# waffcloud/sitewhere

Hardware: AMD Instinct MI355X
Metric: device_events_per_sec (higher is better)
Workload: dtype fp64/int64 (event values as in the reference; no reduced precision)

## Files before the change

### csrc/hip/swgpu.hip

```cpp
#include <hip/hip_runtime.h>
#include <hsa/hsa.h>
#include <hsa/hsa_ext_amd.h>
#include <stdint.h>
#include "swtypes.h"
#include "swdecode.h"
#include "swengine.h"
#include "swseg.h"
#include "swblock.h"

#define BLK 256
#define WAVES (BLK / 64)
#define TILE_ITEMS 4
#define TILE (BLK * TILE_ITEMS)
#define MAX_GRID 2048
#define STAGE_BYTES (32 * 1024)
#define MAX_PROBE 4096

#ifndef SW_XCD_REMAP
#define SW_XCD_REMAP 0
#endif
__device__ __forceinline__ uint32_t sw_block_id() {
#if SW_XCD_REMAP
  const uint32_t nwg = gridDim.x, orig = blockIdx.x, x = orig % 8u, q = nwg / 8u, r = nwg % 8u;
  return (x < r ? x * (q + 1u) : r * (q + 1u) + (x - r) * q) + orig / 8u;
// ... 114 lines not shown
    uint32_t tc, tv;
    const uint32_t pc = block_excl_scan(e ? 1u : 0u, &tc, lds);
    const uint32_t pv = block_excl_scan(v, &tv, lds);
    if (e && run_c + pc < n_msgs) {
      const uint32_t off = run_v + pv;
      msg_off[run_c + pc] = off < raw_bytes ? off : raw_bytes;
    }
    run_c += tc;
    run_v += tv;
  }
}

__device__ __forceinline__ bool stage_window(const uint8_t* __restrict__ raw, const uint32_t* __restrict__ off,
                                             int64_t n_msgs, uint8_t* lds, uint32_t* base_abs) {
  const int64_t m0 = (int64_t)BID * BLK;
  int64_t m1 = m0 + BLK;
  if (m1 > n_msgs) m1 = n_msgs;
  const uint32_t s = off[m0], e = off[m1];
  const uint32_t a0 = s & ~15u;
  const uint32_t span = e - a0;
  if (span > STAGE_BYTES) return false;
  const uint32_t nvec = (span + 15) >> 4;
  const uint4* src = reinterpret_cast<const uint4*>(raw + a0);
  uint4* dst = reinterpret_cast<uint4*>(lds);
  for (uint32_t v = threadIdx.x; v < nvec; v += BLK) dst[v] = src[v];
  __syncthreads();
  *base_abs = a0;
  return true;
}

#define CNT_ERR 0x80000000u
#define CNT_OVR 0x40000000u

__global__ __launch_bounds__(BLK) void k_decode_count(const uint8_t* __restrict__ raw, const uint32_t* __restrict__ off,
                                                      int64_t n_msgs, uint32_t* __restrict__ cnt,
                                                      uint32_t* __restrict__ tsum, SwEngineArgs a) {
  __shared__ __attribute__((aligned(16))) uint8_t lds[STAGE_BYTES];
  if (BID == 0 && threadIdx.x == 0) {
    *a.n_new_names = 0;
    *a.overflow = 0;
    ((ull*)a.stats)[SW_STAT_MSGS] += (ull)a.n_msgs;
  }
  uint32_t base = 0;
  const bool staged = stage_window(raw, off, n_msgs, lds, &base);
  __shared__ uint32_t red[WAVES + 1];
  const int64_t m = (int64_t)BID * BLK + threadIdx.x;
  uint32_t c = 0;
  if (m < n_msgs) {
    uint32_t verdict = SW_DEC_UNKNOWN;
    c = staged ? sw_decode_payload(lds, off[m] - base, off[m + 1] - base, base, 0, 0, nullptr, 0, &verdict)
               : sw_decode_payload(raw, off[m], off[m + 1], 0, 0, 0, nullptr, 0, &verdict);
    cnt[m] = c | (verdict == SW_DEC_ERROR ? CNT_ERR : 0u) | (verdict == SW_DEC_OVERSIZE ? CNT_OVR : 0u);
  }
  uint32_t tot;
  block_excl_scan(c, &tot, red);
  if (threadIdx.x == 0) tsum[BID] = tot;
}

__device__ __forceinline__ void note_name(const SwEventRec& r, ull* __restrict__ key, int64_t mask,
                                          SwNameRef* __restrict__ list, uint32_t* __restrict__ n_list, int64_t cap) {
  if (r.name_hash == 0 || r.etype >= 16) return;
  const ull h = r.name_hash;
  int64_t slot = (int64_t)(h & (ull)mask);
  for (int64_t p = 0; p <= mask && p < MAX_PROBE; ++p) {
    ull old = key[slot];
    if (old == h) return;
    if (old == 0) {
      old = atomicCAS(&key[slot], 0ull, h);
      if (old == 0) {
        const uint32_t k = atomicAdd(n_list, 1u);
        if (k < cap) {
          SwNameRef ref;
          ref.hash = h; ref.off = r.aux_off; ref.len = r.aux_len; ref.src_rank = r.src_rank; ref.pad = r.etype;
          list[k] = ref;
        } else {
          atomicExch(&key[slot], 0ull);
        }
        return;
      }
      if (old == h) return;
    }
    slot = (slot + 1) & mask;
  }
}

__global__ __launch_bounds__(BLK) void k_decode_emit(SwEngineArgs a) {
  __shared__ __attribute__((aligned(16))) uint8_t lds[STAGE_BYTES];
  uint32_t base = 0;
  const bool staged = stage_window(a.raw, a.msg_off, a.n_msgs, lds, &base);
  __shared__ uint32_t red[WAVES + 1];
  const int64_t m = (int64_t)BID * BLK + threadIdx.x;
  uint32_t tot;
  const uint32_t cv = m < a.n_msgs ? a.msg_cnt[m] : 0u;
  const uint32_t pre = block_excl_scan(cv & ~(CNT_ERR | CNT_OVR), &tot, red);
  const uint32_t blk_off = block_sum_prefix(a.msg_evoff, BID, red);
  if (BID == 0) {
    const uint32_t all = block_sum_prefix(a.msg_evoff, gridDim.x, red);
    if (threadIdx.x == 0) *a.n_recs = all;
  }
  if (m >= a.n_msgs) return;
  uint32_t verdict = (cv & CNT_ERR) ? SW_DEC_ERROR : (cv & CNT_OVR) ? SW_DEC_OVERSIZE : SW_DEC_VALID;
  const int64_t o = (int64_t)blk_off + pre;
  if (o >= a.rec_cap) return;
  const uint32_t room = (uint32_t)((a.rec_cap - o) < 0xffffffffll ? (a.rec_cap - o) : 0xffffffffll);
  SwEventRec* out = a.recs + o;
  uint32_t n;
  SwStrRef* sp = a.spans ? a.spans + o : nullptr;
  if (staged)
    n = sw_decode_payload(lds, a.msg_off[m] - base, a.msg_off[m + 1] - base, base, a.now_ms, (uint8_t)a.rank, out, room,
                          &verdict, sp);
  else
    n = sw_decode_payload(a.raw, a.msg_off[m], a.msg_off[m + 1], 0, a.now_ms, (uint8_t)a.rank, out, room, &verdict, sp);
  for (uint32_t k = 0; k < n && k < room; ++k)
    note_name(out[k], (ull*)a.seen_key, a.seen_mask, a.new_names, a.n_new_names, a.names_cap);
}

__global__ void k_decode_end(SwEngineArgs a) {
  if (threadIdx.x == 0 && BID == 0) {
    if (*a.n_recs > a.rec_cap) *a.n_recs = (uint32_t)a.rec_cap;
    ((ull*)a.stats)[SW_STAT_NEW_NAMES] += *a.n_new_names;
  }
}

__device__ __forceinline__ uint32_t part_dest(const SwEngineArgs& a, const SwEventRec& r, uint32_t world,
                                              uint32_t rank) {
  if (r.etype >= 16) return rank;
  int64_t slot = (int64_t)(r.fp_lo & (ull)a.reg_mask);
  for (int64_t p = 0; p <= a.reg_mask && p < MAX_PROBE; ++p) {
    const ulonglong2 k = *reinterpret_cast<const ulonglong2*>(&a.reg[slot].lo);
    if (k.x == r.fp_lo && k.y == r.fp_hi) return a.reg[slot].asg >= 0 ? sw_owner(r.fp_hi, world) : rank;
    if (k.x == 0 && k.y == 0) break;
    slot = (slot + 1) & a.reg_mask;
  }
  return rank;
}

// ... 1095 lines not shown
    run += tot;
  }
}

__global__ void k_presence(SwEngineArgs a) {
  const SwStepParams P = *a.sp;
  if (P.presence_missing_ms <= 0) return;
  const ull limit = (ull)(P.now_ms - P.presence_missing_ms);
  for (int64_t s = (int64_t)BID * BLK + threadIdx.x; s < a.n_asg; s += (int64_t)gridDim.x * BLK) {
    SwAsgState* st = &a.st[s];
    const ull last = st->last;
    const bool miss = last != 0 && last < limit && st->missing == 0 && a.asg_active[s];
    if (!miss) continue;
    st->missing = (ull)P.now_ms;
    const uint32_t g = atomicAdd(a.n_gen, 1u);
    if (g < a.gen_cap) {
      SwEventRec r;
      r.fp_lo = 0; r.fp_hi = 0; r.event_date = P.now_ms; r.name_hash = a.presence_name_hash;
      r.v0 = 0; r.v1 = 0; r.v2 = 0; r.alt_hash = 0;
      r.aux_off = 0; r.aux2_off = 0; r.aux_len = 0; r.aux2_len = 0;
      r.etype = SW_EV_STATE_CHANGE; r.flags = 0; r.src_rank = (uint8_t)a.rank; r.level = 0;
      a.gen[g] = r;
      a.gen_dev[g] = a.asg_ctx[s].device;
      a.gen_asg[g] = (int32_t)s;
    }
  }
}

__global__ void k_decode_begin(SwEngineArgs a) {
  if (threadIdx.x == 0 && BID == 0) {
    *a.n_new_names = 0;
    *a.overflow = 0;
    ((ull*)a.stats)[SW_STAT_MSGS] += (ull)a.n_msgs;
  }
}

__global__ void k_gen_clamp(SwEngineArgs a, uint32_t* gen_rules) {
  if (threadIdx.x == 0 && BID == 0) {
    if (*a.n_gen > a.gen_cap) *a.n_gen = (uint32_t)a.gen_cap;
    if (gen_rules) *gen_rules = *a.n_gen;
  }
}

__global__ void k_step_end(SwEngineArgs a, const uint32_t* n_rule_alerts) {
  if (threadIdx.x == 0 && BID == 0) {
    if (*a.n_gen > a.gen_cap) *a.n_gen = (uint32_t)a.gen_cap;
    *a.store_cursor += (int64_t)*a.n_ok + *a.n_gen;
    *a.n_out = (uint32_t)(*a.store_cursor - *a.step_cursor0);
    *a.seq_base += *a.n_work;
    ull* st = (ull*)a.stats;
    st[SW_STAT_EVENTS] += *a.n_work;
    st[SW_STAT_PERSISTED] += *a.n_out;
    st[SW_STAT_RULE_ALERTS] += *n_rule_alerts;
    st[SW_STAT_PRESENCE] += *a.n_gen - *n_rule_alerts;
    int64_t* meta = a.dd_meta;
    if (meta[2] == 1) {
      meta[0] ^= 1;
      meta[1] = 0;
      meta[2] = 2;
    }
    meta[3] = 0;
    if (a.dd_ff && a.dd_ff_meta[6] >= a.dd_ff_meta[2]) {
      int64_t* fm = a.dd_ff_meta;
      fm[0] = (fm[0] + 1) % a.dd_ff_gens;
      fm[SW_FF_META + fm[0]] = *a.store_cursor;
      fm[6] = 0;
// ... 769 lines not shown
  return n > 0 ? (int)hipMemcpyAsync(dst, src, (size_t)n, hipMemcpyHostToDevice, s) : 0;
}
int sw_memset_async(void* dst, int32_t v, int64_t n, hipStream_t s) {
  return n > 0 ? (int)hipMemsetAsync(dst, v, (size_t)n, s) : 0;
}

int sw_step_snapshot(const uint32_t* scalars, const uint32_t* seg_meta, const uint32_t* rej_cnt,
                     const uint32_t* n_carry, int32_t produced, SwStepSnapshot* host, hipStream_t s) {
  k_step_snapshot<<<1, 64, 0, s>>>(scalars, seg_meta, rej_cnt, n_carry, produced, host);
  return (int)hipGetLastError();
}

int sw_frame_varint(const uint8_t* lens, int64_t nbytes, int64_t n_msgs, uint32_t* msg_off, uint32_t raw_bytes,
                    uint32_t* tmp, int64_t tmp_len, hipStream_t s) {
  int64_t nt = (nbytes + TILE - 1) / TILE;
  if (nt < 1) nt = 1;
  if (2 * nt > tmp_len) return -2;
  if (nbytes <= 0 || n_msgs <= 0) return (int)hipMemsetAsync(msg_off, 0, sizeof(uint32_t) * (n_msgs + 1), s);
  uint32_t* tcnt = tmp;
  uint32_t* tlen = tmp + nt;
  k_vlen_tiles<<<(unsigned)nt, BLK, 0, s>>>(lens, nbytes, tcnt, tlen);
  k_vlen_apply<<<(unsigned)nt, BLK, 0, s>>>(lens, nbytes, tcnt, tlen, msg_off, n_msgs, raw_bytes);
  return (int)hipGetLastError();
}

int sw_phase_decode(const SwEngineArgs* ap, hipStream_t s) {
  const SwEngineArgs a = *ap;
  if (a.n_msgs <= 0) {
    k_decode_begin<<<1, 64, 0, s>>>(a);
    (void)hipMemsetAsync(a.n_recs, 0, sizeof(uint32_t), s);
    return (int)hipGetLastError();
  }
  const unsigned nb = (unsigned)((a.n_msgs + BLK - 1) / BLK);
  k_decode_count<<<nb, BLK, 0, s>>>(a.raw, a.msg_off, a.n_msgs, a.msg_cnt, a.msg_evoff, a);
  k_decode_emit<<<nb, BLK, 0, s>>>(a);
  if (a.world > 1) k_decode_end<<<1, 64, 0, s>>>(a);
  return (int)hipGetLastError();
}

int sw_phase_partition(const SwEngineArgs* ap, hipStream_t s) {
  const SwEngineArgs a = *ap;
  const int64_t ntiles = (a.carry_cap + a.rec_cap + TILE - 1) / TILE;
  if (a.world > 64 || ntiles * a.world > a.part_tmp_len || !a.carry || !a.n_carry || !a.spill || !a.n_spill ||
      a.carry == a.spill || !a.part_owner || !a.part_bytes || !a.part_meta || ntiles >= 0x7fffffff)
    return -3;
  if (a.send_str && (!a.part_len || !a.carry_spans || !a.carry_str || !a.spill_spans || !a.spill_str ||
                     a.carry_str == a.spill_str || a.carry_str_cap <= 0 || a.carry_str_cap > 0xffffffffll ||
                     a.str_cap > 0x7fffffffll))
    return -4;
  k_part_count<<<(unsigned)ntiles, BLK, 0, s>>>(a.carry, a.n_carry, a.recs, a.n_recs, (int)a.world, (int)a.rank,
                                                a.part_tmp, ntiles, a);
  int rc = launch_scan(a.part_tmp, ntiles * a.world, a.part_tmp + ntiles * a.world, nullptr, a.scan_tmp,
                       a.scan_tmp_len, s);
  if (rc) return rc;
  const uint32_t* toff = a.part_tmp + ntiles * a.world;
  k_part_cut<<<(unsigned)a.world, BLK, 0, s>>>(toff, a.part_tmp, ntiles, a.n_carry, a.n_recs, a);
  k_part_write<<<(unsigned)ntiles, BLK, 0, s>>>(a.carry, a.n_carry, a.recs, a.n_recs, (int)a.world, (int)a.rank, toff,
                                                a.part_tmp, ntiles, a.send, a.shuf_cap, a.spill, a.carry_cap, a);
  k_part_counts<<<1, 64, 0, s>>>(toff, a.part_tmp, ntiles, (int)a.world, a);
  return (int)hipGetLastError();
}

int sw_phase_unpack(const SwEngineArgs* ap, hipStream_t s) {
  const SwEngineArgs a = *ap;
  if (a.work_str && (a.str_cap & 15)) return -5;
  k_unpack<<<grid_for(a.rec_cap), BLK, 0, s>>>(a.recv, a.recv_cnt, (int)a.world, a.shuf_cap, a.work, a.n_work,
                                               a.rec_cap, a);
  return (int)hipGetLastError();
}

// ... 464 lines not shown
```

### csrc/include/swdecode.h

```cpp
#pragma once
#include "swtypes.h"

SW_HD void sw_fill_control(SwEventRec* r, uint8_t etype, uint32_t abs_start, uint32_t abs_end,
                           uint64_t lo, uint64_t hi, int64_t now_ms, uint8_t src_rank) {
  r->fp_lo = lo; r->fp_hi = hi; r->event_date = now_ms; r->name_hash = 0;
  r->v0 = 0; r->v1 = 0; r->v2 = 0; r->alt_hash = 0;
  r->aux_off = abs_start; r->aux2_off = abs_end; r->aux_len = 0; r->aux2_len = 0;
  r->etype = etype; r->flags = 0; r->src_rank = src_rank; r->level = 0;
}

SW_HD void sw_clear_span(SwStrRef* s) {
  s->alt_off = 0; s->meta_off = 0; s->alt_len = 0; s->meta_len = 0; s->k = 0; s->has = 0; s->pad = 0;
}

SW_HD bool sw_read_tag(const uint8_t* buf, uint32_t* pos, uint32_t end, uint32_t* f, uint32_t* wt) {
  uint64_t key;
  if (!sw_read_varint(buf, pos, end, &key) || key > 0xffffffffull || (key >> 3) == 0) return false;
  *f = (uint32_t)(key >> 3);
  *wt = (uint32_t)(key & 7);
  return true;
}

SW_HD bool sw_check_pair(const uint8_t* buf, uint32_t* pos, uint32_t end, uint32_t wt2, uint32_t* len1 = nullptr) {
  uint64_t len;
  if (!sw_read_varint(buf, pos, end, &len) || len > (uint64_t)(end - *pos)) return false;
  uint32_t p = *pos;
  const uint32_t e = p + (uint32_t)len;
  bool h1 = false, h2 = false;
  while (p < e) {
    uint32_t f, wt;
    if (!sw_read_tag(buf, &p, e, &f, &wt)) return false;
    const uint32_t vs = p;
    if (!sw_skip_field(buf, &p, e, wt)) return false;
    if (f == 1 && wt == 2) {
      h1 = true;
      if (len1) {
        uint32_t q = vs;
        uint64_t l;
        sw_read_varint(buf, &q, e, &l);
        if ((uint32_t)l > *len1) *len1 = (uint32_t)l;
      }
    }
    h2 |= f == 2 && wt == wt2;
  }
  *pos = e;
  return h1 && h2;
}

#define SW_DEC_UNKNOWN 0u
#define SW_DEC_VALID 1u
#define SW_DEC_ERROR 2u
#define SW_DEC_OVERSIZE 3u
SW_HD uint32_t sw_decode_payload(const uint8_t* buf, uint32_t start, uint32_t end, uint32_t abs_base,
                                 int64_t now_ms, uint8_t src_rank, SwEventRec* out, uint32_t max_out,
                                 uint32_t* verdict = nullptr, SwStrRef* spans = nullptr) {
  const uint32_t known = verdict ? *verdict : SW_DEC_UNKNOWN;
  if (out && known == SW_DEC_ERROR) {
    if (max_out) {
      sw_fill_control(out, SW_EV_DECODE_ERROR, abs_base + start, abs_base + end, 0, 0, now_ms, src_rank);
      if (spans) sw_clear_span(spans);
    }
    return 1;
  }
  const bool trusted = out && known == SW_DEC_VALID;
  uint32_t pos = start;
  uint64_t hlen = 0, blen = 0, v = 0;
  uint64_t cmd = 0;
  bool ok = sw_read_varint(buf, &pos, end, &hlen) && hlen <= (uint64_t)(end - pos);
  if (ok) {
    uint32_t hend = pos + (uint32_t)hlen;
    while (ok && pos < hend) {
      uint32_t f, wt;
      ok = sw_read_tag(buf, &pos, hend, &f, &wt);
      if (!ok) break;
      if (f == 1 && wt == 0) {
        ok = sw_read_varint(buf, &pos, hend, &v);
        if (v >= 1 && v <= 8) cmd = v;
      } else {
        ok = sw_skip_field(buf, &pos, hend, wt);
      }
    }
    ok = ok && sw_read_varint(buf, &pos, end, &blen) && blen <= (uint64_t)(end - pos);
  }
  if (!ok || cmd < 1 || cmd > 8) {
    if (out && max_out) {
      sw_fill_control(out, SW_EV_DECODE_ERROR, abs_base + start, abs_base + end, 0, 0, now_ms, src_rank);
      if (spans) sw_clear_span(spans);
    }
    if (!out && verdict) *verdict = SW_DEC_ERROR;
    return 1;
  }
  const uint32_t bstart = pos, bend = pos + (uint32_t)blen;
  const bool event = cmd == SW_CMD_SEND_DEVICE_MEASUREMENTS || cmd == SW_CMD_SEND_DEVICE_LOCATION ||
                     cmd == SW_CMD_SEND_DEVICE_ALERT;
  const uint32_t meta_f = cmd == SW_CMD_SEND_DEVICE_MEASUREMENTS ? 4u : cmd == SW_CMD_SEND_DEVICE_LOCATION ? 6u : 5u;

  uint64_t lo = 0, hi = 0, date = 0;
  bool has_dev = false, has_date = false, has_us = false, us = false, has_elev = false, has_alt = false;
  bool req_a = false, req_b = false;
  uint32_t n_mx = 0, name_max = 0;
  double lat = 0, lon = 0, elev = 0;
  uint32_t t_off = start, t_len = 0, m_off = start, m_len = 0;
  uint32_t a_off = start, a_len = 0;
  uint32_t md_lo = 0, md_hi = 0;
  bool has_md = false;
  pos = bstart;
  while (ok && pos < bend) {
    uint32_t f, wt;
    const uint32_t fstart = pos;
    ok = sw_read_tag(buf, &pos, bend, &f, &wt);
    if (!ok) break;
    if (f == 1 && wt == 2) {
      ok = sw_read_varint(buf, &pos, bend, &v) && v <= (uint64_t)(bend - pos);
      if (!ok) break;
      if (out) sw_fingerprint(buf + pos, (uint32_t)v, &lo, &hi);
      has_dev = true;
      pos += (uint32_t)v;
      continue;
    }
    if (f == SW_FIELD_ALTERNATE_ID && wt == 2 && event) {
      ok = sw_read_varint(buf, &pos, bend, &v) && v <= (uint64_t)(bend - pos);
      if (!ok) break;
      a_off = pos; a_len = (uint32_t)v; has_alt = true;
      pos += (uint32_t)v;
      continue;
    }
    if (event && f == meta_f && wt == 2) {
      ok = trusted ? sw_skip_field(buf, &pos, bend, wt) : sw_check_pair(buf, &pos, bend, 2);
      if (!has_md) md_lo = fstart;
      md_hi = pos;
      has_md = true;
      continue;
    }
    switch (cmd) {
      case SW_CMD_SEND_DEVICE_MEASUREMENTS:
        if (f == 2 && wt == 2) { n_mx++; ok = trusted ? sw_skip_field(buf, &pos, bend, wt) : sw_check_pair(buf, &pos, bend, 1, &name_max); }
        else if (f == 3 && wt == 1) { if (pos + 8 > bend) { ok = false; break; } date = sw_load_le64(buf + pos); pos += 8; has_date = true; }
        else if (f == 5 && wt == 0) { ok = sw_read_varint(buf, &pos, bend, &v); has_us = true; us = v != 0; }
        else ok = sw_skip_field(buf, &pos, bend, wt);
        break;
      case SW_CMD_SEND_DEVICE_LOCATION:
        if ((f == 2 || f == 3 || f == 4 || f == 5) && wt == 1) {
          if (pos + 8 > bend) { ok = false; break; }
          uint64_t bits = sw_load_le64(buf + pos); pos += 8;
          double d;
          __builtin_memcpy(&d, &bits, 8);
          if (f == 2) { lat = d; req_a = true; } else if (f == 3) { lon = d; req_b = true; }
          else if (f == 4) { elev = d; has_elev = true; }
          else { date = bits; has_date = true; }
        } else if (f == 7 && wt == 0) { ok = sw_read_varint(buf, &pos, bend, &v); has_us = true; us = v != 0; }
        else ok = sw_skip_field(buf, &pos, bend, wt);
        break;
      case SW_CMD_SEND_DEVICE_ALERT:
        if ((f == 2 || f == 3) && wt == 2) {
          ok = sw_read_varint(buf, &pos, bend, &v) && v <= (uint64_t)(bend - pos);
          if (!ok) break;
          if (f == 2) { t_off = pos; t_len = (uint32_t)v; req_a = true; } else { m_off = pos; m_len = (uint32_t)v; req_b = true; }
          pos += (uint32_t)v;
        } else if (f == 4 && wt == 1) { if (pos + 8 > bend) { ok = false; break; } date = sw_load_le64(buf + pos); pos += 8; has_date = true; }
        else if (f == 6 && wt == 0) { ok = sw_read_varint(buf, &pos, bend, &v); has_us = true; us = v != 0; }
        else ok = sw_skip_field(buf, &pos, bend, wt);
        break;
      default:
        ok = sw_skip_field(buf, &pos, bend, wt);
        break;
    }
  }
  if ((cmd == SW_CMD_SEND_DEVICE_LOCATION || cmd == SW_CMD_SEND_DEVICE_ALERT) && !(req_a && req_b)) ok = false;
  if (!ok || !has_dev) {
    if (!out && verdict) *verdict = SW_DEC_ERROR;
    if (out && max_out) {
      sw_fill_control(out, SW_EV_DECODE_ERROR, abs_base + start, abs_base + end, 0, 0, now_ms, src_rank);
      if (spans) sw_clear_span(spans);
    }
    return 1;
  }
  const bool oversize = event && (known == SW_DEC_OVERSIZE ||
                                  (!trusted && (a_len > 0xffffu || md_hi - md_lo > 0xffffu || t_len > 0xffffu ||
                                                m_len > 0xffffu || name_max > 0xffffu)));
  if (oversize) {
    if (!out && verdict) *verdict = SW_DEC_OVERSIZE;
    if (!out) return 1;
    if (!max_out) return 0;
    sw_fill_control(out, SW_EV_OVERSIZE, abs_base + start, abs_base + end, lo, hi, now_ms, src_rank);
    if (spans) sw_clear_span(spans);
    return 1;
  }
  uint8_t flags = (has_us ? SW_F_HAS_UPDATE_STATE : 0) | (us ? SW_F_UPDATE_STATE : 0) |
                  (has_date ? SW_F_HAS_DATE : 0) | (has_elev ? SW_F_HAS_ELEVATION : 0);
  int64_t edate = has_date ? (int64_t)date : now_ms;
  SwStrRef sp;
  sp.alt_off = abs_base + a_off; sp.alt_len = (uint16_t)a_len;
  sp.meta_off = has_md ? abs_base + md_lo : abs_base + start; sp.meta_len = has_md ? (uint16_t)(md_hi - md_lo) : 0;
  sp.k = 0; sp.has = (has_alt ? SW_SR_ALT : 0) | (has_md ? SW_SR_META : 0); sp.pad = 0;

  if (!out && verdict) *verdict = SW_DEC_VALID;
  if (!out) return cmd == SW_CMD_SEND_DEVICE_MEASUREMENTS ? n_mx : 1;
  const uint64_t alt = has_alt && (cmd != SW_CMD_SEND_DEVICE_MEASUREMENTS || n_mx == 1) ? sw_hash64(buf + a_off, a_len) : 0;
  if (cmd == SW_CMD_SEND_DEVICE_MEASUREMENTS) {
    if (n_mx > max_out) {
      if (max_out) {
        sw_fill_control(out, SW_EV_DECODE_ERROR, abs_base + start, abs_base + end, lo, hi, now_ms, src_rank);
        if (spans) sw_clear_span(spans);
      }
      return max_out ? 1 : 0;
    }
    const bool multi = n_mx > 1;
    uint32_t k = 0;
    pos = bstart;
    while (pos < bend && k < n_mx) {
      uint64_t key;
      if (!sw_read_varint(buf, &pos, bend, &key)) break;
      uint32_t f = (uint32_t)(key >> 3), wt = (uint32_t)(key & 7);
      if (!(f == 2 && wt == 2)) { if (!sw_skip_field(buf, &pos, bend, wt)) break; continue; }
      sw_read_varint(buf, &pos, bend, &v);
      uint32_t mend = pos + (uint32_t)v;
      uint32_t n_off = start, n_len = 0;
      double val = 0;
      while (pos < mend) {
        uint64_t k2;
        if (!sw_read_varint(buf, &pos, mend, &k2)) { pos = mend; break; }
        uint32_t f2 = (uint32_t)(k2 >> 3), w2 = (uint32_t)(k2 & 7);
        if (f2 == 1 && w2 == 2) {
          uint64_t l2;
          if (!sw_read_varint(buf, &pos, mend, &l2) || l2 > (uint64_t)(mend - pos)) { pos = mend; break; }
          n_off = pos; n_len = (uint32_t)l2; pos += (uint32_t)l2;
        } else if (f2 == 2 && w2 == 1 && pos + 8 <= mend) {
          uint64_t bits = sw_load_le64(buf + pos); pos += 8;
          __builtin_memcpy(&val, &bits, 8);
        } else if (!sw_skip_field(buf, &pos, mend, w2)) { pos = mend; break; }
      }
      pos = mend;
      SwEventRec* r = out + k;
      r->fp_lo = lo; r->fp_hi = hi; r->event_date = edate;
      r->name_hash = n_len ? sw_hash64(buf + n_off, n_len) : 0;
      r->v0 = val; r->v1 = 0; r->v2 = 0;
      r->alt_hash = !has_alt ? 0 : multi ? sw_hash64_sfx(buf + a_off, a_len, k) : alt;
      r->aux_off = abs_base + n_off; r->aux2_off = 0;
      r->aux_len = (uint16_t)n_len; r->aux2_len = 0;
      r->etype = SW_EV_MEASUREMENT; r->flags = flags; r->src_rank = src_rank; r->level = 0;
      if (spans) {
        spans[k] = sp;
        spans[k].k = (uint16_t)(k > 0xffffu ? 0xffffu : k);
        spans[k].has |= multi ? SW_SR_MULTI : 0;
      }
      ++k;
    }
    for (; k < n_mx; ++k) {
      sw_fill_control(out + k, SW_EV_DECODE_ERROR, abs_base + start, abs_base + end, lo, hi, now_ms, src_rank);
      if (spans) sw_clear_span(spans + k);
    }
    return n_mx;
  }
  if (!max_out) return 0;
  if (spans) *spans = sp;
  if (cmd == SW_CMD_SEND_DEVICE_LOCATION) {
    out->fp_lo = lo; out->fp_hi = hi; out->event_date = edate; out->name_hash = 0;
    out->v0 = lat; out->v1 = lon; out->v2 = elev; out->alt_hash = alt;
    out->aux_off = abs_base + start; out->aux2_off = 0; out->aux_len = 0; out->aux2_len = 0;
    out->etype = SW_EV_LOCATION; out->flags = flags; out->src_rank = src_rank; out->level = 0;
    return 1;
  }
  if (cmd == SW_CMD_SEND_DEVICE_ALERT) {
    out->fp_lo = lo; out->fp_hi = hi; out->event_date = edate;
    out->name_hash = t_len ? sw_hash64(buf + t_off, t_len) : 0;
    out->v0 = 0; out->v1 = 0; out->v2 = 0; out->alt_hash = alt;
    out->aux_off = abs_base + t_off; out->aux2_off = abs_base + m_off;
    out->aux_len = (uint16_t)t_len;
    out->aux2_len = (uint16_t)m_len;
    out->etype = SW_EV_ALERT; out->flags = flags; out->src_rank = src_rank; out->level = 0;
    return 1;
  }
  if (spans) sw_clear_span(spans);
  uint8_t et = cmd == SW_CMD_SEND_REGISTRATION ? SW_EV_REGISTRATION
             : cmd == SW_CMD_SEND_ACKNOWLEDGEMENT ? SW_EV_ACK
             : cmd == SW_CMD_SEND_DEVICE_STREAM ? SW_EV_STREAM_CREATE
             : cmd == SW_CMD_SEND_DEVICE_STREAM_DATA ? SW_EV_STREAM_DATA
             : SW_EV_STREAM_DATA_REQUEST;
  sw_fill_control(out, et, abs_base + start, abs_base + end, lo, hi, now_ms, src_rank);
  return 1;
}
```

### sitewhere_amd/_native.py

```python
from __future__ import annotations

import ctypes
import os
import shutil
import subprocess
import threading
from pathlib import Path

ROOT = Path(__file__).resolve().parent.parent
LIB_DIR = Path(__file__).resolve().parent / "_lib"
CSRC = ROOT / "csrc"
GPU_ARCH = os.environ.get("SW_GPU_ARCH", "gfx950")

_NATIVE_SRC = [CSRC / "native" / "swnative.cpp", CSRC / "native" / "swcpuengine.cpp", CSRC / "native" / "swseg.cpp",
               CSRC / "native" / "swindex.cpp", CSRC / "native" / "swroute.cpp", CSRC / "native" / "swsandbox.cpp", CSRC / "native" / "swjson.cpp",
               CSRC / "native" / "swrowjson.cpp"]
_GPU_SRC = [CSRC / "hip" / "swgpu.hip", CSRC / "hip" / "swseg.hip", CSRC / "hip" / "swindex.hip"]
_HEADERS = sorted((CSRC / "include").glob("*.h")) + sorted((CSRC / "hip").glob("*.h"))

_lock = threading.Lock()
_native = None
_gpu = None


# ... 222 lines not shown
            _proto(lib, "swlog_append_routed", c_int64, P, P, P, c_int64, P, P, c_int64, P)
            _proto(lib, "swlog_append", c_int64, P, c_int32, c_int32, P, c_int64, P, c_int64, c_int64)
            _proto(lib, "swlog_end_offset", c_int64, P, c_int32, c_int32)
            _proto(lib, "swlog_begin_offset", c_int64, P, c_int32, c_int32)
            _proto(lib, "swlog_read", c_int64, P, c_int32, c_int32, c_int64, c_int64, P, c_int64, P)
            _proto(lib, "swlog_commit", c_int32, P, c_char_p, c_int32, c_int32, c_int64)
            _proto(lib, "swlog_committed", c_int64, P, c_char_p, c_int32, c_int32)
            _proto(lib, "swlog_append_external", c_int64, P, c_int32, c_int32, P, c_int64, c_int64, c_int64,
                   c_int64)
            _proto(lib, "swlog_view", c_int32, P, c_int32, c_int32, c_int64, P, P, P)
            _proto(lib, "swlog_hold", c_int32, P, c_int32, c_int32, c_int64)
            _proto(lib, "swlog_take_released", c_int64, P, P, c_int64)
            _proto(lib, "sw_partition_for_key", c_int32, c_char_p, c_int32, c_int32)
            _native_gil = lib
    return _native_gil


def gpu():
    global _gpu
    if _gpu is not None:
        return _gpu
    import torch

    with _lock:
        if _gpu is not None:
            return _gpu
        override = os.environ.get("SW_GPU_LIB")
        path = Path(override) if override else LIB_DIR / "libswgpu.so"
        if not override and _stale(path, _GPU_SRC):
            build_gpu()
        lib = ctypes.CDLL(str(path))
        P = c_void_p
        _proto(lib, "sw_phase_decode", c_int32, P, P)
        _proto(lib, "sw_phase_partition", c_int32, P, P)
        _proto(lib, "sw_phase_unpack", c_int32, P, P)
        _proto(lib, "sw_phase_process", c_int32, P, P, P)
        _proto(lib, "sw_pip_batch", c_int32, P, c_int64, P, P, c_int64, P, P)
        _proto(lib, "sw_store_filter", c_int32, P, c_int32, P, c_int64, P, P)
        _proto(lib, "sw_store_series_count", c_int32, P, P, P, P)
        _proto(lib, "sw_store_series", c_int32, P, P, P, c_int64, P, P, c_int64, P, P, P, P, P)
        _proto(lib, "sw_store_near", c_int32, P, P, P, c_int64, P, P)
        _proto(lib, "sw_store_zone", c_int32, P, P, c_int64, P, P)
        _proto(lib, "sw_store_grid", c_int32, P, P, P, P)
        _proto(lib, "sw_grid_lds_cells", c_int64, c_int64)
        _proto(lib, "sw_store_rank", c_int32, P, P, P, P, P, P)
        _proto(lib, "sw_rank_lds_keys", c_int64, c_int64)
        _proto(lib, "sw_rank_combine", c_int32, c_int32)
        _proto(lib, "sw_scan_u32", c_int32, P, c_int64, P, P, P, c_int64, P)
        _proto(lib, "sw_state_lookup", c_int32, P, c_int64, c_int32, c_int32, P, P, P)
        _proto(lib, "sw_abi_sizes", c_int32, P)
        _proto(lib, "sw_host_alloc", c_int32, c_int64, P, P)
        _proto(lib, "sw_host_free", c_int32, P)
        _proto(lib, "sw_push_out", c_int32, P, P, P, c_int64, c_int32, P)
        _proto(lib, "sw_copy_d2h", c_int32, P, P, c_int64, P)
        _proto(lib, "sw_sdma_copy", c_int32, P, P, c_int64, c_int32, ctypes.POINTER(ctypes.c_uint64))
        _proto(lib, "sw_sdma_h2d", c_int32, P, P, c_int64, c_int32, ctypes.POINTER(ctypes.c_uint64))
        _proto(lib, "sw_frame_varint", c_int32, P, c_int64, c_int64, P, ctypes.c_uint32, P, c_int64, P)
        _proto(lib, "sw_set_step_params", c_int32, P, c_int64, c_int64, c_int64, P, P, c_int64, P)
        _proto(lib, "sw_graph_capture_process", c_int32, P, P, c_int32, P, ctypes.POINTER(ctypes.c_void_p))
        _proto(lib, "sw_graph_launch", c_int32, P, P)
        _proto(lib, "sw_graph_destroy", c_int32, P)
        _proto(lib, "sw_sdma_wait", c_int32, c_uint64)
        _proto(lib, "sw_seg_encode", c_int32, P, P, P, P, P, c_int64, P, c_int64, P)
        _proto(lib, "sw_seg_encode_stamped", c_int32, P, P, P, P, P, c_int64, P, c_int64, P, P)
        _proto(lib, "sw_seg_encode_snap", c_int32, P, P, P, P, P, c_int64, P, c_int64, P, P, P, P, P)
        _proto(lib, "sw_seg_aux", c_int32, P, P, P, P, P, c_int64, P, P, c_int64, P)
# ... 52 lines not shown
```

### sitewhere_amd/pipeline/gpu_engine.py

```python
from __future__ import annotations

import ctypes
import functools
import os
import time

import numpy as np
import torch

from .._native import gpu_gil as gpu_lib
from ..models.columnar import (EVENT_REC, RANK_CELL, RANK_QUERY, GRID_CELL, GRID_QUERY_F64, GRID_WORDS, N_STATS, NEAR_QUERY, NEAR_QUERY_F64,
                               OUT_REC, NAME_REF, OUT_REC_SIZE, RING_QUERY, SC_N_GEN, SC_N_NEW_NAMES, SC_N_OK, SC_N_OUT,
                               SC_N_RECS, SC_N_REJ, SC_N_RULE, SC_N_WORK, SC_NAMES, SC_OVERFLOW, SEG_ST_BYTES, SEG_ST_FIRST, SEG_ST_WORDS, SERIES_CELL, SERIES_QUERY,
                               ST_RECHECK, STEP_SNAPSHOT, STR_REF, WIRE_REC, ZONE_QUERY, ZONE_QUERY_F64)
from ..ops.engine_abi import SwEngineArgs
from .config import EngineConfig
from .bus_io import host_view
from .engine_base import EngineBase, StepResult
from .pinned_pool import PinnedPool

_ALIGN = 64
_I64 = np.iinfo(np.int64)


# ... 565 lines not shown

    def string_drops(self) -> dict:
        v = self.t["str_drops"].cpu().numpy()
        return {"oversize": int(v[0])}

    def scalars(self) -> dict:
        v = self.t["scalars"][:len(SC_NAMES)].cpu().numpy()
        return {name: int(x) for name, x in zip(SC_NAMES, v)}

    def step(self, raw: np.ndarray, offs: np.ndarray, now_ms: int, presence: bool | None = None) -> StepResult:
        n_msgs = len(offs) - 1
        with self._lock:
            self._no_framed_pending()
            raw_dev, off_dev = self._stage(raw, offs)
            do_presence = self.presence_due(now_ms) if presence is None else presence
            sel = self.step_async(raw_dev, off_dev, n_msgs, now_ms, presence=do_presence, out_to_device=True)
            self._sync_streams()
            return self._with_block(self.collect(sel, raw, from_device=True), sel, now_ms)

    def decode_only(self, raw: np.ndarray, offs: np.ndarray, now_ms: int, spans: bool = False):
        n_msgs = len(offs) - 1
        with self._lock:
            self._no_framed_pending()
            raw_dev, off_dev = self._stage(raw, offs)
            self._set_batch(raw_dev, off_dev, n_msgs, now_ms)
            _chk(self.lib.sw_phase_decode(ctypes.byref(self.args), self._stream()), "sw_phase_decode")
            self._sync_streams()
            n = min(int(self.t["scalars"][SC_N_RECS].item()), self.cfg.rec_cap)
            recs = self.t["recs"][:n * EVENT_REC.itemsize].cpu().numpy().view(EVENT_REC).copy()
            if not spans:
                return recs
            return recs, self.t["spans"][:n * STR_REF.itemsize].cpu().numpy().view(STR_REF).copy()

    def step_framed(self, batch, now_ms: int, presence: bool | None = None) -> StepResult:
        if batch.lens is None:
            return EngineBase.step_framed(self, batch, now_ms, presence)
        import warnings
        n, nb, nl = batch.n_msgs, len(batch.payload), len(batch.lens)
        if n > self.cfg.max_msgs:
            raise ValueError(f"batch of {n} payloads exceeds EngineConfig.max_msgs={self.cfg.max_msgs}")
        if nb < batch.payload_bytes + _ALIGN:
            raise ValueError("raw batch payload lacks its tail padding")
        with self._lock:
            self._no_framed_pending()
            dev_r, dev_l, dev_o = self._stg_framed.get(nb, nl)
            with warnings.catch_warnings():
                warnings.simplefilter("ignore", UserWarning)
                pt = torch.frombuffer(batch.payload, dtype=torch.uint8) if nb else None
                lt = torch.frombuffer(batch.lens, dtype=torch.uint8) if nl else None
            if pt is not None:
                dev_r[:nb].copy_(pt, non_blocking=True)
            if lt is not None:
                dev_l[:nl].copy_(lt, non_blocking=True)
            self.frame_varint(dev_l, nl, n, dev_o, batch.payload_bytes)
            do_presence = self.presence_due(now_ms) if presence is None else presence
            sel = self.step_async(dev_r[:nb], dev_o[:n + 1], n, now_ms, presence=do_presence, out_to_device=True)
            self._sync_streams()
            return self._with_block(self.collect(sel, np.asarray(batch.payload), from_device=True), sel, now_ms)

    encode_blocks = False
    block_boot = 0

    def _with_block(self, res: StepResult, sel: int, now_ms: int) -> StepResult:
        if self.encode_blocks:
            res.block = self.encode_block(now_ms, res, slot=sel, boot=self.block_boot)
        return res
# ... 1125 lines not shown
```

Before: 536.5 million.

## Speculatively emit single-event records in decode count pass to skip re-decode

Splits the payload decoder into a parse step and an emit step. When the previous batch produced one event per message (tracked through a flag word in device memory), the first pass writes each record directly at index m. The second pass then re-decodes only the messages whose final offset differs, and skips LDS staging for blocks with no remaining work. This avoids decoding every payload twice in the common case. In exchange it adds an extra begin kernel launch, flag bookkeeping across batches, and wasted speculative writes when the batch is mixed.

```diff
diff --git a/csrc/hip/swgpu.hip b/csrc/hip/swgpu.hip
--- a/csrc/hip/swgpu.hip
+++ b/csrc/hip/swgpu.hip
@@ -170,29 +170,10 @@
 #define CNT_ERR 0x80000000u
 #define CNT_OVR 0x40000000u
 
-__global__ __launch_bounds__(BLK) void k_decode_count(const uint8_t* __restrict__ raw, const uint32_t* __restrict__ off,
-                                                      int64_t n_msgs, uint32_t* __restrict__ cnt,
-                                                      uint32_t* __restrict__ tsum, SwEngineArgs a) {
-  __shared__ __attribute__((aligned(16))) uint8_t lds[STAGE_BYTES];
-  if (BID == 0 && threadIdx.x == 0) {
-    *a.n_new_names = 0;
-    *a.overflow = 0;
-    ((ull*)a.stats)[SW_STAT_MSGS] += (ull)a.n_msgs;
-  }
-  uint32_t base = 0;
-  const bool staged = stage_window(raw, off, n_msgs, lds, &base);
-  __shared__ uint32_t red[WAVES + 1];
-  const int64_t m = (int64_t)BID * BLK + threadIdx.x;
-  uint32_t c = 0;
-  if (m < n_msgs) {
-    uint32_t verdict = SW_DEC_UNKNOWN;
-    c = staged ? sw_decode_payload(lds, off[m] - base, off[m + 1] - base, base, 0, 0, nullptr, 0, &verdict)
-               : sw_decode_payload(raw, off[m], off[m + 1], 0, 0, 0, nullptr, 0, &verdict);
-    cnt[m] = c | (verdict == SW_DEC_ERROR ? CNT_ERR : 0u) | (verdict == SW_DEC_OVERSIZE ? CNT_OVR : 0u);
-  }
-  uint32_t tot;
-  block_excl_scan(c, &tot, red);
-  if (threadIdx.x == 0) tsum[BID] = tot;
+#define SPEC_CUR_OFF 1u
+#define SPEC_NEXT_OFF 2u
+__device__ __forceinline__ bool decode_speculates(const SwEngineArgs& a) {
+  return a.str_drops && !(__atomic_load_n(&a.str_drops[1], __ATOMIC_RELAXED) & SPEC_CUR_OFF);
 }
 
 __device__ __forceinline__ void note_name(const SwEventRec& r, ull* __restrict__ key, int64_t mask,
@@ -222,24 +203,69 @@
   }
 }
 
-__global__ __launch_bounds__(BLK) void k_decode_emit(SwEngineArgs a) {
+__global__ __launch_bounds__(BLK) void k_decode_first(const uint8_t* __restrict__ raw, const uint32_t* __restrict__ off,
+                                                      int64_t n_msgs, uint32_t* __restrict__ cnt,
+                                                      uint32_t* __restrict__ tsum, SwEngineArgs a) {
   __shared__ __attribute__((aligned(16))) uint8_t lds[STAGE_BYTES];
+  const bool spec = decode_speculates(a);
   uint32_t base = 0;
-  const bool staged = stage_window(a.raw, a.msg_off, a.n_msgs, lds, &base);
+  const bool staged = stage_window(raw, off, n_msgs, lds, &base);
   __shared__ uint32_t red[WAVES + 1];
   const int64_t m = (int64_t)BID * BLK + threadIdx.x;
+  uint32_t c = 0;
+  if (!spec) {
+    if (m < n_msgs) {
+      uint32_t verdict = SW_DEC_UNKNOWN;
+      c = staged ? sw_decode_payload(lds, off[m] - base, off[m + 1] - base, base, 0, 0, nullptr, 0, &verdict)
+                 : sw_decode_payload(raw, off[m], off[m + 1], 0, 0, 0, nullptr, 0, &verdict);
+      cnt[m] = c | (verdict == SW_DEC_ERROR ? CNT_ERR : 0u) | (verdict == SW_DEC_OVERSIZE ? CNT_OVR : 0u);
+    }
+  } else if (m < n_msgs) {
+    uint32_t verdict = SW_DEC_UNKNOWN;
+    SwEventRec* out = m < a.rec_cap ? a.recs + m : nullptr;
+    SwStrRef* sp = out && a.spans ? a.spans + m : nullptr;
+    c = staged ? sw_decode_once(lds, off[m] - base, off[m + 1] - base, base, a.now_ms, (uint8_t)a.rank, out, &verdict, sp)
+               : sw_decode_once(raw, off[m], off[m + 1], 0, a.now_ms, (uint8_t)a.rank, out, &verdict, sp);
+    cnt[m] = c | (verdict == SW_DEC_ERROR ? CNT_ERR : 0u) | (verdict == SW_DEC_OVERSIZE ? CNT_OVR : 0u);
+    if (out && c == 1) note_name(*out, (ull*)a.seen_key, a.seen_mask, a.new_names, a.n_new_names, a.names_cap);
+  }
+  uint32_t tot;
+  block_excl_scan(c, &tot, red);
+  if (threadIdx.x == 0) tsum[BID] = tot;
+}
+
+__global__ __launch_bounds__(BLK) void k_decode_second(SwEngineArgs a) {
+  __shared__ __attribute__((aligned(16))) uint8_t lds[STAGE_BYTES];
+  __shared__ uint32_t red[WAVES + 1];
+  const int64_t m = (int64_t)BID * BLK + threadIdx.x;
+  const bool spec = decode_speculates(a);
+  uint32_t base = 0;
+  bool staged = false;
+  if (!spec) staged = stage_window(a.raw, a.msg_off, a.n_msgs, lds, &base);
   uint32_t tot;
   const uint32_t cv = m < a.n_msgs ? a.msg_cnt[m] : 0u;
-  const uint32_t pre = block_excl_scan(cv & ~(CNT_ERR | CNT_OVR), &tot, red);
+  const uint32_t c = cv & ~(CNT_ERR | CNT_OVR);
+  const uint32_t pre = block_excl_scan(c, &tot, red);
   const uint32_t blk_off = block_sum_prefix(a.msg_evoff, BID, red);
   if (BID == 0) {
     const uint32_t all = block_sum_prefix(a.msg_evoff, gridDim.x, red);
-    if (threadIdx.x == 0) *a.n_recs = all;
-  }
-  if (m >= a.n_msgs) return;
+    if (threadIdx.x == 0) {
+      *a.n_recs = all;
+      if (a.str_drops) {
+        const uint32_t w = __atomic_load_n(&a.str_drops[1], __ATOMIC_RELAXED) & SPEC_CUR_OFF;
+        __atomic_store_n(&a.str_drops[1], w | ((int64_t)all == a.n_msgs ? 0u : SPEC_NEXT_OFF), __ATOMIC_RELAXED);
+      }
+    }
+  }
+  const int64_t o = (int64_t)blk_off + pre;
+  const bool in_place = spec && c == 1 && o == m && m < a.rec_cap;
+  const bool todo = m < a.n_msgs && !in_place && o < a.rec_cap;
+  if (spec) {
+    if (!__syncthreads_or(todo)) return;
+    staged = stage_window(a.raw, a.msg_off, a.n_msgs, lds, &base);
+  }
+  if (!todo) return;
   uint32_t verdict = (cv & CNT_ERR) ? SW_DEC_ERROR : (cv & CNT_OVR) ? SW_DEC_OVERSIZE : SW_DEC_VALID;
-  const int64_t o = (int64_t)blk_off + pre;
-  if (o >= a.rec_cap) return;
   const uint32_t room = (uint32_t)((a.rec_cap - o) < 0xffffffffll ? (a.rec_cap - o) : 0xffffffffll);
   SwEventRec* out = a.recs + o;
   uint32_t n;
@@ -1401,6 +1427,10 @@
     *a.n_new_names = 0;
     *a.overflow = 0;
     ((ull*)a.stats)[SW_STAT_MSGS] += (ull)a.n_msgs;
+    if (a.str_drops) {
+      const uint32_t nxt = a.str_drops[1] & SPEC_NEXT_OFF;
+      a.str_drops[1] = nxt | (nxt ? SPEC_CUR_OFF : 0u);
+    }
   }
 }
 
@@ -2236,10 +2266,16 @@
     return (int)hipGetLastError();
   }
   const unsigned nb = (unsigned)((a.n_msgs + BLK - 1) / BLK);
-  k_decode_count<<<nb, BLK, 0, s>>>(a.raw, a.msg_off, a.n_msgs, a.msg_cnt, a.msg_evoff, a);
-  k_decode_emit<<<nb, BLK, 0, s>>>(a);
+  k_decode_begin<<<1, 64, 0, s>>>(a);
+  k_decode_first<<<nb, BLK, 0, s>>>(a.raw, a.msg_off, a.n_msgs, a.msg_cnt, a.msg_evoff, a);
+  k_decode_second<<<nb, BLK, 0, s>>>(a);
   if (a.world > 1) k_decode_end<<<1, 64, 0, s>>>(a);
   return (int)hipGetLastError();
+}
+
+int sw_decode_set_speculation(const SwEngineArgs* ap, int32_t on, hipStream_t s) {
+  if (!ap->str_drops) return -3;
+  return (int)hipMemsetD32Async((hipDeviceptr_t)(ap->str_drops + 1), on ? 0 : (int)SPEC_NEXT_OFF, 1, s);
 }
 
 int sw_phase_partition(const SwEngineArgs* ap, hipStream_t s) {
diff --git a/csrc/include/swdecode.h b/csrc/include/swdecode.h
--- a/csrc/include/swdecode.h
+++ b/csrc/include/swdecode.h
@@ -51,18 +51,28 @@
 #define SW_DEC_VALID 1u
 #define SW_DEC_ERROR 2u
 #define SW_DEC_OVERSIZE 3u
-SW_HD uint32_t sw_decode_payload(const uint8_t* buf, uint32_t start, uint32_t end, uint32_t abs_base,
-                                 int64_t now_ms, uint8_t src_rank, SwEventRec* out, uint32_t max_out,
-                                 uint32_t* verdict = nullptr, SwStrRef* spans = nullptr) {
-  const uint32_t known = verdict ? *verdict : SW_DEC_UNKNOWN;
-  if (out && known == SW_DEC_ERROR) {
-    if (max_out) {
-      sw_fill_control(out, SW_EV_DECODE_ERROR, abs_base + start, abs_base + end, 0, 0, now_ms, src_rank);
-      if (spans) sw_clear_span(spans);
-    }
-    return 1;
-  }
-  const bool trusted = out && known == SW_DEC_VALID;
+
+typedef struct SwParsed {
+  uint32_t verdict;
+  uint32_t cmd;
+  uint32_t bstart, bend;
+  uint32_t dev_off, dev_len;
+  uint32_t n_mx;
+  uint32_t t_off, t_len, m_off, m_len;
+  uint32_t a_off, a_len;
+  uint32_t md_lo, md_hi;
+  uint64_t date;
+  double lat, lon, elev;
+  uint8_t flags;
+  bool has_alt, has_md, has_date;
+} SwParsed;
+
+SW_HD uint32_t sw_parsed_count(const SwParsed* p) {
+  return p->verdict == SW_DEC_VALID && p->cmd == SW_CMD_SEND_DEVICE_MEASUREMENTS ? p->n_mx : 1u;
+}
+
+SW_HD uint32_t sw_parse_payload(const uint8_t* buf, uint32_t start, uint32_t end, uint32_t known, bool trusted,
+                                SwParsed* p) {
   uint32_t pos = start;
   uint64_t hlen = 0, blen = 0, v = 0;
   uint64_t cmd = 0;
@@ -82,24 +92,18 @@
     }
     ok = ok && sw_read_varint(buf, &pos, end, &blen) && blen <= (uint64_t)(end - pos);
   }
-  if (!ok || cmd < 1 || cmd > 8) {
-    if (out && max_out) {
-      sw_fill_control(out, SW_EV_DECODE_ERROR, abs_base + start, abs_base + end, 0, 0, now_ms, src_rank);
-      if (spans) sw_clear_span(spans);
-    }
-    if (!out && verdict) *verdict = SW_DEC_ERROR;
-    return 1;
-  }
+  if (!ok || cmd < 1 || cmd > 8) return p->verdict = SW_DEC_ERROR;
   const uint32_t bstart = pos, bend = pos + (uint32_t)blen;
   const bool event = cmd == SW_CMD_SEND_DEVICE_MEASUREMENTS || cmd == SW_CMD_SEND_DEVICE_LOCATION ||
                      cmd == SW_CMD_SEND_DEVICE_ALERT;
   const uint32_t meta_f = cmd == SW_CMD_SEND_DEVICE_MEASUREMENTS ? 4u : cmd == SW_CMD_SEND_DEVICE_LOCATION ? 6u : 5u;
 
-  uint64_t lo = 0, hi = 0, date = 0;
+  uint64_t date = 0;
   bool has_dev = false, has_date = false, has_us = false, us = false, has_elev = false, has_alt = false;
   bool req_a = false, req_b = false;
   uint32_t n_mx = 0, name_max = 0;
   double lat = 0, lon = 0, elev = 0;
+  uint32_t d_off = start, d_len = 0;
   uint32_t t_off = start, t_len = 0, m_off = start, m_len = 0;
   uint32_t a_off = start, a_len = 0;
   uint32_t md_lo = 0, md_hi = 0;
@@ -113,8 +117,7 @@
     if (f == 1 && wt == 2) {
       ok = sw_read_varint(buf, &pos, bend, &v) && v <= (uint64_t)(bend - pos);
       if (!ok) break;
-      if (out) sw_fingerprint(buf + pos, (uint32_t)v, &lo, &hi);
-      has_dev = true;
+      d_off = pos; d_len = (uint32_t)v; has_dev = true;
       pos += (uint32_t)v;
       continue;
     }
@@ -167,35 +170,49 @@
     }
   }
   if ((cmd == SW_CMD_SEND_DEVICE_LOCATION || cmd == SW_CMD_SEND_DEVICE_ALERT) && !(req_a && req_b)) ok = false;
-  if (!ok || !has_dev) {
-    if (!out && verdict) *verdict = SW_DEC_ERROR;
-    if (out && max_out) {
-      sw_fill_control(out, SW_EV_DECODE_ERROR, abs_base + start, abs_base + end, 0, 0, now_ms, src_rank);
-      if (spans) sw_clear_span(spans);
-    }
-    return 1;
-  }
+  if (!ok || !has_dev) return p->verdict = SW_DEC_ERROR;
+  p->cmd = (uint32_t)cmd; p->bstart = bstart; p->bend = bend;
+  p->dev_off = d_off; p->dev_len = d_len; p->n_mx = n_mx;
+  p->t_off = t_off; p->t_len = t_len; p->m_off = m_off; p->m_len = m_len;
+  p->a_off = a_off; p->a_len = a_len; p->md_lo = md_lo; p->md_hi = md_hi;
+  p->date = date; p->lat = lat; p->lon = lon; p->elev = elev;
+  p->flags = (uint8_t)((has_us ? SW_F_HAS_UPDATE_STATE : 0) | (us ? SW_F_UPDATE_STATE : 0) |
+                       (has_date ? SW_F_HAS_DATE : 0) | (has_elev ? SW_F_HAS_ELEVATION : 0));
+  p->has_alt = has_alt; p->has_md = has_md; p->has_date = has_date;
   const bool oversize = event && (known == SW_DEC_OVERSIZE ||
                                   (!trusted && (a_len > 0xffffu || md_hi - md_lo > 0xffffu || t_len > 0xffffu ||
                                                 m_len > 0xffffu || name_max > 0xffffu)));
-  if (oversize) {
-    if (!out && verdict) *verdict = SW_DEC_OVERSIZE;
-    if (!out) return 1;
-    if (!max_out) return 0;
+  return p->verdict = oversize ? SW_DEC_OVERSIZE : SW_DEC_VALID;
+}
+
+SW_HD uint32_t sw_emit_parsed(const uint8_t* buf, uint32_t start, uint32_t end, uint32_t abs_base, int64_t now_ms,
+                              uint8_t src_rank, const SwParsed* p, SwEventRec* out, uint32_t max_out,
+                              SwStrRef* spans = nullptr) {
+  if (p->verdict == SW_DEC_ERROR) {
+    if (max_out) {
+      sw_fill_control(out, SW_EV_DECODE_ERROR, abs_base + start, abs_base + end, 0, 0, now_ms, src_rank);
+      if (spans) sw_clear_span(spans);
+    }
+    return 1;
+  }
+  const uint32_t cmd = p->cmd;
+  if (!max_out && (p->verdict == SW_DEC_OVERSIZE || cmd != SW_CMD_SEND_DEVICE_MEASUREMENTS)) return 0;
+  uint64_t lo = 0, hi = 0;
+  sw_fingerprint(buf + p->dev_off, p->dev_len, &lo, &hi);
+  if (p->verdict == SW_DEC_OVERSIZE) {
     sw_fill_control(out, SW_EV_OVERSIZE, abs_base + start, abs_base + end, lo, hi, now_ms, src_rank);
     if (spans) sw_clear_span(spans);
     return 1;
   }
-  uint8_t flags = (has_us ? SW_F_HAS_UPDATE_STATE : 0) | (us ? SW_F_UPDATE_STATE : 0) |
-                  (has_date ? SW_F_HAS_DATE : 0) | (has_elev ? SW_F_HAS_ELEVATION : 0);
-  int64_t edate = has_date ? (int64_t)date : now_ms;
+  const bool has_alt = p->has_alt, has_md = p->has_md;
+  const uint32_t a_off = p->a_off, a_len = p->a_len, n_mx = p->n_mx;
+  const uint8_t flags = p->flags;
+  const int64_t edate = p->has_date ? (int64_t)p->date : now_ms;
   SwStrRef sp;
   sp.alt_off = abs_base + a_off; sp.alt_len = (uint16_t)a_len;
-  sp.meta_off = has_md ? abs_base + md_lo : abs_base + start; sp.meta_len = has_md ? (uint16_t)(md_hi - md_lo) : 0;
+  sp.meta_off = has_md ? abs_base + p->md_lo : abs_base + start; sp.meta_len = has_md ? (uint16_t)(p->md_hi - p->md_lo) : 0;
   sp.k = 0; sp.has = (has_alt ? SW_SR_ALT : 0) | (has_md ? SW_SR_META : 0); sp.pad = 0;
 
-  if (!out && verdict) *verdict = SW_DEC_VALID;
-  if (!out) return cmd == SW_CMD_SEND_DEVICE_MEASUREMENTS ? n_mx : 1;
   const uint64_t alt = has_alt && (cmd != SW_CMD_SEND_DEVICE_MEASUREMENTS || n_mx == 1) ? sw_hash64(buf + a_off, a_len) : 0;
   if (cmd == SW_CMD_SEND_DEVICE_MEASUREMENTS) {
     if (n_mx > max_out) {
@@ -206,8 +223,9 @@
       return max_out ? 1 : 0;
     }
     const bool multi = n_mx > 1;
-    uint32_t k = 0;
-    pos = bstart;
+    const uint32_t bend = p->bend;
+    uint32_t k = 0, pos = p->bstart;
+    uint64_t v = 0;
     while (pos < bend && k < n_mx) {
       uint64_t key;
       if (!sw_read_varint(buf, &pos, bend, &key)) break;
@@ -252,22 +270,22 @@
     }
     return n_mx;
   }
-  if (!max_out) return 0;
-  if (spans) *spans = sp;
   if (cmd == SW_CMD_SEND_DEVICE_LOCATION) {
+    if (spans) *spans = sp;
     out->fp_lo = lo; out->fp_hi = hi; out->event_date = edate; out->name_hash = 0;
-    out->v0 = lat; out->v1 = lon; out->v2 = elev; out->alt_hash = alt;
+    out->v0 = p->lat; out->v1 = p->lon; out->v2 = p->elev; out->alt_hash = alt;
     out->aux_off = abs_base + start; out->aux2_off = 0; out->aux_len = 0; out->aux2_len = 0;
     out->etype = SW_EV_LOCATION; out->flags = flags; out->src_rank = src_rank; out->level = 0;
     return 1;
   }
   if (cmd == SW_CMD_SEND_DEVICE_ALERT) {
+    if (spans) *spans = sp;
     out->fp_lo = lo; out->fp_hi = hi; out->event_date = edate;
-    out->name_hash = t_len ? sw_hash64(buf + t_off, t_len) : 0;
+    out->name_hash = p->t_len ? sw_hash64(buf + p->t_off, p->t_len) : 0;
     out->v0 = 0; out->v1 = 0; out->v2 = 0; out->alt_hash = alt;
-    out->aux_off = abs_base + t_off; out->aux2_off = abs_base + m_off;
-    out->aux_len = (uint16_t)t_len;
-    out->aux2_len = (uint16_t)m_len;
+    out->aux_off = abs_base + p->t_off; out->aux2_off = abs_base + p->m_off;
+    out->aux_len = (uint16_t)p->t_len;
+    out->aux2_len = (uint16_t)p->m_len;
     out->etype = SW_EV_ALERT; out->flags = flags; out->src_rank = src_rank; out->level = 0;
     return 1;
   }
@@ -280,3 +298,26 @@
   sw_fill_control(out, et, abs_base + start, abs_base + end, lo, hi, now_ms, src_rank);
   return 1;
 }
+
+SW_HD uint32_t sw_decode_payload(const uint8_t* buf, uint32_t start, uint32_t end, uint32_t abs_base,
+                                 int64_t now_ms, uint8_t src_rank, SwEventRec* out, uint32_t max_out,
+                                 uint32_t* verdict = nullptr, SwStrRef* spans = nullptr) {
+  const uint32_t known = verdict ? *verdict : SW_DEC_UNKNOWN;
+  SwParsed p;
+  if (out && known == SW_DEC_ERROR) p.verdict = SW_DEC_ERROR;
+  else sw_parse_payload(buf, start, end, known, out && known == SW_DEC_VALID, &p);
+  if (!out) {
+    if (verdict) *verdict = p.verdict;
+    return sw_parsed_count(&p);
+  }
+  return sw_emit_parsed(buf, start, end, abs_base, now_ms, src_rank, &p, out, max_out, spans);
+}
+
+SW_HD uint32_t sw_decode_once(const uint8_t* buf, uint32_t start, uint32_t end, uint32_t abs_base, int64_t now_ms,
+                              uint8_t src_rank, SwEventRec* out, uint32_t* verdict, SwStrRef* spans = nullptr) {
+  SwParsed p;
+  *verdict = sw_parse_payload(buf, start, end, SW_DEC_UNKNOWN, false, &p);
+  const uint32_t n = sw_parsed_count(&p);
+  if (n == 1 && out) sw_emit_parsed(buf, start, end, abs_base, now_ms, src_rank, &p, out, 1, spans);
+  return n;
+}
diff --git a/sitewhere_amd/_native.py b/sitewhere_amd/_native.py
--- a/sitewhere_amd/_native.py
+++ b/sitewhere_amd/_native.py
@@ -278,6 +278,8 @@
         lib = ctypes.CDLL(str(path))
         P = c_void_p
         _proto(lib, "sw_phase_decode", c_int32, P, P)
+        if not override or hasattr(lib, "sw_decode_set_speculation"):
+            _proto(lib, "sw_decode_set_speculation", c_int32, P, c_int32, P)
         _proto(lib, "sw_phase_partition", c_int32, P, P)
         _proto(lib, "sw_phase_unpack", c_int32, P, P)
         _proto(lib, "sw_phase_process", c_int32, P, P, P)
diff --git a/sitewhere_amd/pipeline/gpu_engine.py b/sitewhere_amd/pipeline/gpu_engine.py
--- a/sitewhere_amd/pipeline/gpu_engine.py
+++ b/sitewhere_amd/pipeline/gpu_engine.py
@@ -621,6 +621,11 @@
                 return recs
             return recs, self.t["spans"][:n * STR_REF.itemsize].cpu().numpy().view(STR_REF).copy()
 
+    def set_decode_speculation(self, on: bool) -> None:
+        with self._lock:
+            _chk(self.lib.sw_decode_set_speculation(ctypes.byref(self.args), 1 if on else 0, self._stream()),
+                 "sw_decode_set_speculation")
+
     def step_framed(self, batch, now_ms: int, presence: bool | None = None) -> StepResult:
         if batch.lens is None:
             return EngineBase.step_framed(self, batch, now_ms, presence)
```

After: 427.0 million. -20.4%, worse.
